# theEricMa/ScaleDreamer

Hardware: AMD Instinct MI355X
Metric: ASD train steps/sec (64x64 render, SD2.1) (higher is better)
Workload: dtype f32 renderer / f16 diffusion (f32 accumulate); 1 GPU; asd_sd_nerf: 1 view/GPU, 64x64 rays, 512 spp occgrid march, implicit-volume iNGP (16x2 hash grid 2^19, MLP 64), SD-2.1 UNet batch 5 (CFG+Perp-Neg+shifted t), VAE 512^2 fwd+bwd, AdamW; views_per_gpu=1, parallelism=dp1, diffusion_backend=hip, diffusion_weights=seeded random init (seed 1)

## Files before the change

scaledreamer_amd/csrc/nn_ops.hip:

```cpp
#include "asd_common.h"
#include <type_traits>

typedef _Float16 half_t;
typedef half_t half8 __attribute__((ext_vector_type(8)));

__device__ __forceinline__ float silu_f(float v) { return asd_silu_fast(v); }
__device__ __forceinline__ float gelu_f(float x) { return 0.5f * x * (1.f + erff(x * 0.70710678118654752440f)); }

#ifndef GN_UNR
#define GN_UNR 4
#endif
#ifndef GN_CAP_A
#define GN_CAP_A 512
#endif
#ifndef GN_FOLD_RECORDS
#define GN_FOLD_RECORDS 96
#endif

__global__ __launch_bounds__(256) void gn_stats_kernel(const half_t* __restrict__ x1, int c1, const half_t* __restrict__ x2,
                                                       int c2, int hw, int rows_per_block, float* __restrict__ stats) {
    __shared__ float gsum[32], gsq[32];
    const int C = c1 + c2, slots = C / 8, cg = C / 32;
    const int b = blockIdx.x, tid = threadIdx.x;
    if (tid < 32) { gsum[tid] = 0.f; gsq[tid] = 0.f; }
    __syncthreads();
    const int r0 = blockIdx.y * rows_per_block, r1 = min(hw, r0 + rows_per_block);
    const int rows_in_flight = slots >= 256 ? 1 : 256 / slots;
    const int rsub = slots >= 256 ? 0 : tid / slots;
    const int slot0 = slots >= 256 ? tid : tid % slots;
#pragma unroll
    for (int j = 0; j < 2; ++j) {
        const int slot = slot0 + j * 256;
        if (slot >= slots || rsub >= rows_in_flight || (j == 1 && slots <= 256)) continue;
        float s[8], q[8];
#pragma unroll
        for (int k = 0; k < 8; ++k) { s[k] = 0.f; q[k] = 0.f; }
        const int c = slot * 8;
        const half_t* base = c < c1 ? x1 + (size_t)b * hw * c1 + c : x2 + (size_t)b * hw * c2 + (c - c1);
        const size_t rstride = c < c1 ? c1 : c2;
        int r = r0 + rsub;
        for (; r + (GN_UNR - 1) * rows_in_flight < r1; r += GN_UNR * rows_in_flight) {
            half8 v[GN_UNR];
#pragma unroll
            for (int u = 0; u < GN_UNR; ++u) v[u] = *(const half8*)(base + (size_t)(r + u * rows_in_flight) * rstride);
#pragma unroll
            for (int u = 0; u < GN_UNR; ++u)
#pragma unroll
                for (int k = 0; k < 8; ++k) { const float f = (float)v[u][k]; s[k] += f; q[k] = fmaf(f, f, q[k]); }
        }
        for (; r < r1; r += rows_in_flight) {
            const half8 v = *(const half8*)(base + (size_t)r * rstride);
#pragma unroll
            for (int k = 0; k < 8; ++k) { const float f = (float)v[k]; s[k] += f; q[k] = fmaf(f, f, q[k]); }
        }
        int g = c / cg;
        float ss = 0.f, qq = 0.f;
#pragma unroll
        for (int k = 0; k < 8; ++k) {
            const int gk = (c + k) / cg;
            if (gk != g) { atomicAdd(&gsum[g], ss); atomicAdd(&gsq[g], qq); g = gk; ss = 0.f; qq = 0.f; }
            ss += s[k]; qq += q[k];
        }
        atomicAdd(&gsum[g], ss);
        atomicAdd(&gsq[g], qq);
    }
    __syncthreads();
    if (tid < 32) {
        float* part = stats + ((size_t)b * gridDim.y + blockIdx.y) * 64;
        part[tid * 2] = gsum[tid];
        part[tid * 2 + 1] = gsq[tid];
    }
}

__device__ __forceinline__ void gn_reduce_partials(const float* __restrict__ partials, int b, int n_chunks, float* st ,
                                                   float (*scratch)[64] ) {
    const int tid = threadIdx.x, v = tid & 63, q = tid >> 6;
    const float* src = partials + (size_t)b * n_chunks * 64 + v;
    float acc[8];
#pragma unroll
    for (int u = 0; u < 8; ++u) acc[u] = 0.f;
    for (int c = q; c < n_chunks; c += 32) {
        float t[8];
#pragma unroll
        for (int u = 0; u < 8; ++u) t[u] = src[(size_t)min(c + 4 * u, n_chunks - 1) * 64];
#pragma unroll
        for (int u = 0; u < 8; ++u) acc[u] += c + 4 * u < n_chunks ? t[u] : 0.f;
    }
    scratch[q][v] = ((acc[0] + acc[1]) + (acc[2] + acc[3])) + ((acc[4] + acc[5]) + (acc[6] + acc[7]));
    __syncthreads();
    if (tid < 64) st[tid] = (scratch[0][tid] + scratch[1][tid]) + (scratch[2][tid] + scratch[3][tid]);
    __syncthreads();
}

template <bool SILU>
__global__ __launch_bounds__(256) void gn_apply_kernel(const half_t* __restrict__ x1, int c1, const half_t* __restrict__ x2,
                                                       int c2, int hw, int rows_per_block, const half_t* __restrict__ gamma,
                                                       const half_t* __restrict__ beta, float eps, float inv_cnt,
                                                       const float* __restrict__ partials, int n_chunks,
                                                       float* __restrict__ stats_out, half_t* __restrict__ y) {
    __shared__ float st[64];
    __shared__ float scratch[4][64];
    const int C = c1 + c2, slots = C / 8, cg = C / 32;
    const int b = blockIdx.x, tid = threadIdx.x;
    const int r0 = blockIdx.y * rows_per_block, r1 = min(hw, r0 + rows_per_block);
    const int rows_in_flight = slots >= 256 ? 1 : 256 / slots;
    const int rsub = slots >= 256 ? 0 : tid / slots;
    const int slot0 = slots >= 256 ? tid : tid % slots;
    const bool act0 = slot0 < slots && rsub < rows_in_flight;
    const int cA = slot0 * 8;
    const half_t* baseA = cA < c1 ? x1 + (size_t)b * hw * c1 + cA : x2 + (size_t)b * hw * c2 + (cA - c1);
    const size_t rstrideA = cA < c1 ? c1 : c2;
    half8 pre[GN_UNR], gpre = {}, bpre = {};
    const int rA = r0 + rsub;
    const bool pre_ok = act0 && rA + (GN_UNR - 1) * rows_in_flight < r1;
    if (act0) { gpre = *(const half8*)(gamma + cA); bpre = *(const half8*)(beta + cA); }
    if (pre_ok) {
#pragma unroll
        for (int u = 0; u < GN_UNR; ++u) pre[u] = *(const half8*)(baseA + (size_t)(rA + u * rows_in_flight) * rstrideA);
    }
    gn_reduce_partials(partials, b, n_chunks, st, scratch);
    if (blockIdx.y == 0 && tid < 64) stats_out[b * 64 + tid] = st[tid];
#pragma unroll
    for (int j = 0; j < 2; ++j) {
        const int slot = slot0 + j * 256;
        if (slot >= slots || rsub >= rows_in_flight || (j == 1 && slots <= 256)) continue;
        const int c = slot * 8;
        half8 gv = gpre, bv = bpre;
        if (j == 1) { gv = *(const half8*)(gamma + c); bv = *(const half8*)(beta + c); }
        float sa[8], sb[8], ta[8], tb[8];
#pragma unroll
        for (int k = 0; k < 8; ++k) {
            const int g = (c + k) / cg;
            const float mean = st[g * 2] * inv_cnt;
            const float var = fmaxf(st[g * 2 + 1] * inv_cnt - mean * mean, 0.f);
            sa[k] = rsqrtf(var + eps) * (float)gv[k];
            sb[k] = (float)bv[k] - mean * sa[k];
            ta[k] = ASD_NEG_LOG2E * sa[k]; tb[k] = ASD_NEG_LOG2E * sb[k];
        }
        const half_t* base = c < c1 ? x1 + (size_t)b * hw * c1 + c : x2 + (size_t)b * hw * c2 + (c - c1);
        const size_t rstride = c < c1 ? c1 : c2;
        half_t* ybase = y + (size_t)b * hw * C + c;
        auto emit = [&](const half8& v, int r) __attribute__((always_inline)) {
            half8 o;
#pragma unroll
            for (int k = 0; k < 8; ++k) {
                const float xf = (float)v[k];
                float f = fmaf(xf, sa[k], sb[k]);
                if (SILU) f *= asd_sigmoid_exp2(fmaf(xf, ta[k], tb[k]));
                o[k] = (half_t)f;
            }
            *(half8*)(ybase + (size_t)r * C) = o;
        };
        int r = r0 + rsub;
        if (j == 0 && pre_ok) {
#pragma unroll
            for (int u = 0; u < GN_UNR; ++u) emit(pre[u], r + u * rows_in_flight);
            r += GN_UNR * rows_in_flight;
        }
        auto trips = [&](auto uc) __attribute__((always_inline)) {
            constexpr int U = decltype(uc)::value;
            for (; r + (U - 1) * rows_in_flight < r1; r += U * rows_in_flight) {
                half8 v[U];
#pragma unroll
                for (int u = 0; u < U; ++u) v[u] = *(const half8*)(base + (size_t)(r + u * rows_in_flight) * rstride);
#pragma unroll
                for (int u = 0; u < U; ++u) emit(v[u], r + u * rows_in_flight);
            }
        };
        trips(std::integral_constant<int, GN_UNR>{});
        trips(std::integral_constant<int, 1>{});
    }
}

__device__ __forceinline__ float silu_grad(float z) { return asd_silu_grad_fast(z); }

#ifndef GN_BWD_UNR
#define GN_BWD_UNR 4
#endif
#ifndef GN_BWD_WIDE_NT
#define GN_BWD_WIDE_NT 512
#endif

template <int NT, bool SILU>
__global__ __launch_bounds__(NT) void gn_bwd_stats_kernel(const half_t* __restrict__ x, const half_t* __restrict__ dy, int C,
                                                           int hw, int rows_per_block, const half_t* __restrict__ gamma,
                                                           const half_t* __restrict__ beta, float eps, float inv_cnt,
                                                           const float* __restrict__ fstats, float* __restrict__ bstats) {
    __shared__ float gsum[32], gsq[32];
    const int slots = C / 8, cg = C / 32;
    const int b = blockIdx.x, tid = threadIdx.x;
    if (tid < 32) { gsum[tid] = 0.f; gsq[tid] = 0.f; }
    __syncthreads();
    const int r0 = blockIdx.y * rows_per_block, r1 = min(hw, r0 + rows_per_block);
    const int rows_in_flight = slots >= NT ? 1 : NT / slots;
    const int rsub = slots >= NT ? 0 : tid / slots;
    const int slot0 = slots >= NT ? tid : tid % slots;
#pragma unroll
    for (int j = 0; j < 2; ++j) {
        const int slot = slot0 + j * NT;
        if (slot >= slots || rsub >= rows_in_flight || (j == 1 && slots <= NT)) continue;
        const int c = slot * 8;
        float rstd[8], nmr[8], gm[8], bt[8], s[8], q[8];
#pragma unroll
        for (int k = 0; k < 8; ++k) {
            const int g = (c + k) / cg;
            const float mean = fstats[(b * 32 + g) * 2] * inv_cnt;
            rstd[k] = rsqrtf(fmaxf(fstats[(b * 32 + g) * 2 + 1] * inv_cnt - mean * mean, 0.f) + eps);
            nmr[k] = -mean * rstd[k];
            gm[k] = (float)gamma[c + k]; bt[k] = (float)beta[c + k];
            s[k] = 0.f; q[k] = 0.f;
        }
        auto accum = [&](const half8& xv, const half8& dv) __attribute__((always_inline)) {
#pragma unroll
            for (int k = 0; k < 8; ++k) {
                const float xh = fmaf((float)xv[k], rstd[k], nmr[k]);
                float g = (float)dv[k] * gm[k];
                if (SILU) g *= silu_grad(fmaf(xh, gm[k], bt[k]));
                s[k] += g;
                q[k] = fmaf(g, xh, q[k]);
            }
        };
        int r = r0 + rsub;
        auto trips = [&](auto uc) __attribute__((always_inline)) {
            constexpr int U = decltype(uc)::value;
            for (; r + (U - 1) * rows_in_flight < r1; r += U * rows_in_flight) {
                half8 xv[U], dv[U];
#pragma unroll
                for (int u = 0; u < U; ++u) {
                    const size_t off = ((size_t)b * hw + r + u * rows_in_flight) * C + c;
                    xv[u] = *(const half8*)(x + off); dv[u] = *(const half8*)(dy + off);
                }
#pragma unroll
                for (int u = 0; u < U; ++u) accum(xv[u], dv[u]);
            }
        };
        trips(std::integral_constant<int, GN_BWD_UNR>{});
        if (GN_BWD_UNR > 2) trips(std::integral_constant<int, 2>{});
        trips(std::integral_constant<int, 1>{});
        int g = c / cg;
        float ss = 0.f, qq = 0.f;
#pragma unroll
        for (int k = 0; k < 8; ++k) {
            const int gk = (c + k) / cg;
            if (gk != g) { atomicAdd(&gsum[g], ss); atomicAdd(&gsq[g], qq); g = gk; ss = 0.f; qq = 0.f; }
            ss += s[k]; qq += q[k];
        }
        atomicAdd(&gsum[g], ss);
        atomicAdd(&gsq[g], qq);
    }
    __syncthreads();
    if (tid < 32) {
        float* part = bstats + ((size_t)b * gridDim.y + blockIdx.y) * 64;
        part[tid * 2] = gsum[tid];
        part[tid * 2 + 1] = gsq[tid];
    }
}

template <bool SILU, bool ADD>
__global__ __launch_bounds__(256) void gn_bwd_apply_kernel(const half_t* __restrict__ x, const half_t* __restrict__ dy, int C,
                                                           int hw, int rows_per_block, const half_t* __restrict__ gamma,
                                                           const half_t* __restrict__ beta, float eps, float inv_cnt,
                                                           const float* __restrict__ fstats, const float* __restrict__ bpartials,
                                                           int n_chunks, const half_t* __restrict__ dx_add,
                                                           half_t* __restrict__ dx) {
    __shared__ float st[64];
    __shared__ float scratch[4][64];
    const int slots = C / 8, cg = C / 32;
    const int b = blockIdx.x, tid = threadIdx.x;
    const int r0 = blockIdx.y * rows_per_block, r1 = min(hw, r0 + rows_per_block);
    const int rows_in_flight = slots >= 256 ? 1 : 256 / slots;
    const int rsub = slots >= 256 ? 0 : tid / slots;
    const int slot0 = slots >= 256 ? tid : tid % slots;
    const bool act0 = slot0 < slots && rsub < rows_in_flight;
    const int cA = slot0 * 8, rA = r0 + rsub;
    const bool pre_ok = act0 && rA + rows_in_flight < r1;
    half8 gpre = {}, bpre = {}, px[2], pd[2], pa[2] = {};
    if (act0) { gpre = *(const half8*)(gamma + cA); bpre = *(const half8*)(beta + cA); }
    if (pre_ok) {
#pragma unroll
        for (int u = 0; u < 2; ++u) {
            const size_t off = ((size_t)b * hw + rA + u * rows_in_flight) * C + cA;
            px[u] = *(const half8*)(x + off); pd[u] = *(const half8*)(dy + off);
            if (ADD) pa[u] = *(const half8*)(dx_add + off);
        }
    }
    gn_reduce_partials(bpartials, b, n_chunks, st, scratch);
#pragma unroll
    for (int j = 0; j < 2; ++j) {
        const int slot = slot0 + j * 256;
        if (slot >= slots || rsub >= rows_in_flight || (j == 1 && slots <= 256)) continue;
        const int c = slot * 8;
        half8 gv = gpre, bv = bpre;
        if (j == 1) { gv = *(const half8*)(gamma + c); bv = *(const half8*)(beta + c); }
        float rstd[8], nmr[8], gm[8], bt[8], G[8], c1[8], c2[8];
#pragma unroll
        for (int k = 0; k < 8; ++k) {
            const int g = (c + k) / cg;
            const float mean = fstats[(b * 32 + g) * 2] * inv_cnt;
            rstd[k] = rsqrtf(fmaxf(fstats[(b * 32 + g) * 2 + 1] * inv_cnt - mean * mean, 0.f) + eps);
            nmr[k] = -mean * rstd[k];
            gm[k] = (float)gv[k]; bt[k] = (float)bv[k];
            G[k] = gm[k] * rstd[k];
            c1[k] = -(st[g * 2] * inv_cnt) * rstd[k]; c2[k] = -(st[g * 2 + 1] * inv_cnt) * rstd[k];
        }
        auto emit = [&](const half8& xv, const half8& dv, const half8& av, int r) __attribute__((always_inline)) {
            half8 o;
#pragma unroll
            for (int k = 0; k < 8; ++k) {
                const float xh = fmaf((float)xv[k], rstd[k], nmr[k]);
                const float lin = fmaf(xh, c2[k], c1[k]);
                float f = SILU ? fmaf((float)dv[k] * G[k], silu_grad(fmaf(xh, gm[k], bt[k])), lin) : fmaf((float)dv[k], G[k], lin);
                if (ADD) f += (float)av[k];
                o[k] = (half_t)f;
            }
            *(half8*)(dx + ((size_t)b * hw + r) * C + c) = o;
        };
        int r = r0 + rsub;
        if (j == 0 && pre_ok) {
            emit(px[0], pd[0], pa[0], r);
            emit(px[1], pd[1], pa[1], r + rows_in_flight);
            r += 2 * rows_in_flight;
        }
        auto trips = [&](auto uc) __attribute__((always_inline)) {
            constexpr int U = decltype(uc)::value;
            for (; r + (U - 1) * rows_in_flight < r1; r += U * rows_in_flight) {
                half8 xv[U], dv[U], av[U] = {};
#pragma unroll
                for (int u = 0; u < U; ++u) {
                    const size_t off = ((size_t)b * hw + r + u * rows_in_flight) * C + c;
                    xv[u] = *(const half8*)(x + off); dv[u] = *(const half8*)(dy + off);
                    if (ADD) av[u] = *(const half8*)(dx_add + off);
                }
#pragma unroll
                for (int u = 0; u < U; ++u) emit(xv[u], dv[u], av[u], r + u * rows_in_flight);
            }
        };
        trips(std::integral_constant<int, GN_BWD_UNR>{});
        if (GN_BWD_UNR > 2) trips(std::integral_constant<int, 2>{});
        trips(std::integral_constant<int, 1>{});
    }
}

__global__ __launch_bounds__(256) void transpose_f16_kernel(const half_t* __restrict__ x, int rows, int cols, int ldx,
                                                            half_t* __restrict__ y, int ldy) {
    __shared__ half_t tile[64][66];
    const int r0 = blockIdx.y * 64, c0 = blockIdx.x * 64;
    for (int q = threadIdx.x; q < 64 * 64; q += 256) {
        const int r = q / 64, c = q % 64;
        tile[r][c] = (r0 + r < rows && c0 + c < cols) ? x[(size_t)(r0 + r) * ldx + c0 + c] : (half_t)0.f;
    }
    __syncthreads();
    for (int q = threadIdx.x; q < 64 * 64; q += 256) {
        const int c = q / 64, r = q % 64;
        if (c0 + c < cols && r0 + r < rows) y[(size_t)(c0 + c) * ldy + r0 + r] = tile[r][c];
    }
}

template <int NV>
__global__ __launch_bounds__(256) void layernorm_kernel(const half_t* __restrict__ x, int rows, int C,
                                                        const half_t* __restrict__ gamma, const half_t* __restrict__ beta,
                                                        float eps, half_t* __restrict__ y) {
    const int lane = threadIdx.x & 63;
    const int wave = blockIdx.x * 4 + (threadIdx.x >> 6), n_waves = gridDim.x * 4;
    half8 gm[NV], bt[NV];
#pragma unroll
    for (int j = 0; j < NV; ++j) {
        const int c = lane * 8 + j * 512;
        if (c < C) { gm[j] = *(const half8*)(gamma + c); bt[j] = *(const half8*)(beta + c); }
    }
    const float inv_c = 1.f / (float)C;
    for (int row = wave; row < rows; row += n_waves) {
        const half_t* xr = x + (size_t)row * C;
        half8 v[NV];
        float s = 0.f;
#pragma unroll
        for (int j = 0; j < NV; ++j) {
            const int c = lane * 8 + j * 512;
            if (c < C) {
                v[j] = *(const half8*)(xr + c);
#pragma unroll
                for (int k = 0; k < 8; ++k) s += (float)v[j][k];
            }
        }
        const float mean = asd_wave_sum(s) * inv_c;
        float q = 0.f;
#pragma unroll
        for (int j = 0; j < NV; ++j)
            if (lane * 8 + j * 512 < C) {
#pragma unroll
                for (int k = 0; k < 8; ++k) { const float d = (float)v[j][k] - mean; q = fmaf(d, d, q); }
            }
        const float rstd = rsqrtf(asd_wave_sum(q) * inv_c + eps);
#pragma unroll
        for (int j = 0; j < NV; ++j) {
            const int c = lane * 8 + j * 512;
            if (c < C) {
                half8 o;
#pragma unroll
                for (int k = 0; k < 8; ++k) o[k] = (half_t)(((float)v[j][k] - mean) * rstd * (float)gm[j][k] + (float)bt[j][k]);
                *(half8*)(y + (size_t)row * C + c) = o;
            }
        }
    }
}


__device__ __forceinline__ float block_reduce(float v, float* red, bool is_max) {
#pragma unroll
    for (int off = 32; off > 0; off >>= 1) {
        const float o = __shfl_xor(v, off, 64);
        v = is_max ? fmaxf(v, o) : v + o;
    }
    const int wave = threadIdx.x >> 6;
    __syncthreads();
    if ((threadIdx.x & 63) == 0) red[wave] = v;
    __syncthreads();
    const float a = red[0], b = red[1], c = red[2], d = red[3];
    return is_max ? fmaxf(fmaxf(a, b), fmaxf(c, d)) : (a + b) + (c + d);
}

template <int NV>
__global__ __launch_bounds__(256) void softmax_kernel(const half_t* __restrict__ x, int ldx, int cols, float scale,
                                                      half_t* __restrict__ y, int ldy) {
    __shared__ float red[4];
    const half_t* xr = x + (size_t)blockIdx.x * ldx;
    half8 v[NV];
    float m = -INFINITY;
#pragma unroll
    for (int j = 0; j < NV; ++j) {
        const int c = threadIdx.x * 8 + j * 2048;
        if (c < cols) {
            v[j] = *(const half8*)(xr + c);
#pragma unroll
            for (int k = 0; k < 8; ++k) m = fmaxf(m, (float)v[j][k]);
        }
    }
    m = block_reduce(m, red, true) * scale;
    float e[NV][8];
    float s = 0.f;
#pragma unroll
    for (int j = 0; j < NV; ++j)
        if (threadIdx.x * 8 + j * 2048 < cols) {
#pragma unroll
            for (int k = 0; k < 8; ++k) { e[j][k] = __expf(fmaf((float)v[j][k], scale, -m)); s += e[j][k]; }
        }
    const float inv = 1.f / block_reduce(s, red, false);
#pragma unroll
    for (int j = 0; j < NV; ++j) {
        const int c = threadIdx.x * 8 + j * 2048;
        if (c < cols) {
            half8 o;
#pragma unroll
            for (int k = 0; k < 8; ++k) o[k] = (half_t)(e[j][k] * inv);
            *(half8*)(y + (size_t)blockIdx.x * ldy + c) = o;
        }
    }
}

template <int NV>
__global__ __launch_bounds__(256) void softmax_bwd_kernel(const half_t* __restrict__ p, const half_t* __restrict__ dp, int ld,
                                                          int cols, float scale, half_t* __restrict__ ds) {
    __shared__ float red[4];
    const size_t base = (size_t)blockIdx.x * ld;
    half8 pv[NV], dv[NV];
    float s = 0.f;
#pragma unroll
    for (int j = 0; j < NV; ++j) {
        const int c = threadIdx.x * 8 + j * 2048;
        if (c < cols) {
            pv[j] = *(const half8*)(p + base + c);
            dv[j] = *(const half8*)(dp + base + c);
#pragma unroll
            for (int k = 0; k < 8; ++k) s = fmaf((float)pv[j][k], (float)dv[j][k], s);
        }
    }
    s = block_reduce(s, red, false);
#pragma unroll
    for (int j = 0; j < NV; ++j) {
        const int c = threadIdx.x * 8 + j * 2048;
        if (c < cols) {
            half8 o;
#pragma unroll
            for (int k = 0; k < 8; ++k) o[k] = (half_t)(scale * (float)pv[j][k] * ((float)dv[j][k] - s));
            *(half8*)(ds + base + c) = o;
        }
    }
}

__global__ __launch_bounds__(256) void geglu_kernel(const half_t* __restrict__ h, int rows, int C, half_t* __restrict__ y) {
    const int slots = C / 8;
    const size_t total = (size_t)rows * slots;
    for (size_t i = (size_t)blockIdx.x * 256 + threadIdx.x; i < total; i += (size_t)gridDim.x * 256) {
        const size_t row = i / slots;
        const int c = (int)(i - row * slots) * 8;
        const half8 a = *(const half8*)(h + row * 2 * C + c), g = *(const half8*)(h + row * 2 * C + C + c);
        half8 o;
#pragma unroll
        for (int k = 0; k < 8; ++k) o[k] = (half_t)((float)a[k] * gelu_f((float)g[k]));
        *(half8*)(y + row * C + c) = o;
    }
}

__global__ __launch_bounds__(256) void silu_kernel(const half_t* __restrict__ x, size_t n8, half_t* __restrict__ y) {
    for (size_t i = (size_t)blockIdx.x * 256 + threadIdx.x; i < n8; i += (size_t)gridDim.x * 256) {
        const half8 v = *(const half8*)(x + i * 8);
        half8 o;
#pragma unroll
        for (int k = 0; k < 8; ++k) o[k] = (half_t)silu_f((float)v[k]);
        *(half8*)(y + i * 8) = o;
    }
}

__global__ void timestep_embedding_kernel(const float* __restrict__ t, int n, int dim, half_t* __restrict__ y) {
    const int i = blockIdx.x * blockDim.x + threadIdx.x;
    const int half = dim / 2;
    if (i >= n * half) return;
    const int r = i / half, k = i - r * half;
    const float freq = expf(-logf(10000.f) * (float)k / (float)half);
    const float a = t[r] * freq;
    y[(size_t)r * dim + k] = (half_t)cosf(a);
    y[(size_t)r * dim + half + k] = (half_t)sinf(a);
}

__global__ __launch_bounds__(256) void concat_kernel(const half_t* __restrict__ x1, int c1, const half_t* __restrict__ x2, int c2,
                                                     size_t rows, half_t* __restrict__ y) {
    const int C = c1 + c2, slots = C / 8;
    const size_t total = rows * slots;
    for (size_t i = (size_t)blockIdx.x * 256 + threadIdx.x; i < total; i += (size_t)gridDim.x * 256) {
        const size_t row = i / slots;
        const int c = (int)(i - row * slots) * 8;
        *(half8*)(y + row * C + c) = c < c1 ? *(const half8*)(x1 + row * c1 + c) : *(const half8*)(x2 + row * c2 + (c - c1));
    }
}

__global__ __launch_bounds__(256) void pad_cast_kernel(const float* __restrict__ x, size_t rows, int c, half_t* __restrict__ y, int c_pad) {
    const size_t total = rows * (size_t)c_pad;
    for (size_t i = (size_t)blockIdx.x * 256 + threadIdx.x; i < total; i += (size_t)gridDim.x * 256) {
        const size_t r = i / c_pad;
        const int j = (int)(i - r * c_pad);
        y[i] = j < c ? (half_t)x[r * c + j] : (half_t)0.f;
    }
}

__global__ __launch_bounds__(1024) void gn_reduce_records_kernel(const float* __restrict__ records, int n, float* __restrict__ out) {
    __shared__ float scratch[16][64];
    const int b = blockIdx.x, S = gridDim.y, per = (n + S - 1) / S;
    const int c0 = blockIdx.y * per, c1 = min(n, c0 + per);
    const int v = threadIdx.x & 63, q = threadIdx.x >> 6;
    const float* src = records + (size_t)b * n * 64 + v;
    float acc[8];
#pragma unroll
    for (int u = 0; u < 8; ++u) acc[u] = 0.f;
    int c = c0 + q;
    for (; c + 7 * 16 < c1; c += 8 * 16) {
        float t[8];
#pragma unroll
        for (int u = 0; u < 8; ++u) t[u] = src[(size_t)(c + u * 16) * 64];
#pragma unroll
        for (int u = 0; u < 8; ++u) acc[u] += t[u];
    }
#pragma unroll
    for (int u = 0; u < 8; ++u)
        if (c + u * 16 < c1) acc[u] += src[(size_t)(c + u * 16) * 64];
    scratch[q][v] = ((acc[0] + acc[1]) + (acc[2] + acc[3])) + ((acc[4] + acc[5]) + (acc[6] + acc[7]));
    __syncthreads();
    if (threadIdx.x < 64) {
        float s = 0.f;
#pragma unroll
        for (int u = 0; u < 16; ++u) s += scratch[u][v];
        out[((size_t)b * S + blockIdx.y) * 64 + v] = s;
    }
}

static int gn_apply_chunks(int hw, int C, int batch) {
    const int slots = C / 8, rif = slots >= 256 ? 1 : 256 / slots;
    const int chunks = asd_div_up(hw, GN_UNR * rif), cap_a = asd_div_up(GN_CAP_A, batch);
    return chunks > cap_a ? cap_a : chunks;
}

__global__ __launch_bounds__(256) void gather_rows_kernel(const uint4* __restrict__ src, const int* __restrict__ idx, size_t row16,
                                                          uint4* __restrict__ dst) {
    const size_t i = blockIdx.y;
    const uint4* s = src + (size_t)idx[i] * row16;
    uint4* d = dst + i * row16;
    for (size_t q = (size_t)blockIdx.x * 256 + threadIdx.x; q < row16; q += (size_t)gridDim.x * 256) d[q] = s[q];
}

static void gn_launch_apply(dim3 grid, hipStream_t s, const void* x1, int c1, const void* x2, int c2, int hw, int rows_per_block,
                            const void* gamma, const void* beta, float eps, int silu, const float* partials, int n_chunks, float* stats,
                            void* y) {
    const float inv_cnt = 1.f / ((float)hw * (float)((c1 + c2) / 32));
#define GN_APPLY_ARGS (const half_t*)x1, c1, (const half_t*)x2, c2, hw, rows_per_block, (const half_t*)gamma, (const half_t*)beta, eps, inv_cnt, \
                      partials, n_chunks, stats, (half_t*)y
    if (silu) hipLaunchKernelGGL(gn_apply_kernel<true>, grid, dim3(256), 0, s, GN_APPLY_ARGS);
    else hipLaunchKernelGGL(gn_apply_kernel<false>, grid, dim3(256), 0, s, GN_APPLY_ARGS);
#undef GN_APPLY_ARGS
}

static void gn_launch_bwd_stats(bool wide, dim3 grid, hipStream_t s, const void* x, const void* dy, int c, int hw, int rows_per_block,
                                const void* gamma, const void* beta, float eps, int silu, const float* fstats, float* bstats) {
    const float inv_cnt = 1.f / ((float)hw * (float)(c / 32));
#define GN_BWD_STATS_ARGS (const half_t*)x, (const half_t*)dy, c, hw, rows_per_block, (const half_t*)gamma, (const half_t*)beta, eps, inv_cnt, fstats, bstats
    if (wide) {
        if (silu) hipLaunchKernelGGL((gn_bwd_stats_kernel<GN_BWD_WIDE_NT, true>), grid, dim3(GN_BWD_WIDE_NT), 0, s, GN_BWD_STATS_ARGS);
        else hipLaunchKernelGGL((gn_bwd_stats_kernel<GN_BWD_WIDE_NT, false>), grid, dim3(GN_BWD_WIDE_NT), 0, s, GN_BWD_STATS_ARGS);
    } else {
        if (silu) hipLaunchKernelGGL((gn_bwd_stats_kernel<256, true>), grid, dim3(256), 0, s, GN_BWD_STATS_ARGS);
        else hipLaunchKernelGGL((gn_bwd_stats_kernel<256, false>), grid, dim3(256), 0, s, GN_BWD_STATS_ARGS);
    }
#undef GN_BWD_STATS_ARGS
}

static void gn_launch_bwd_apply(dim3 grid, hipStream_t s, const void* x, const void* dy, int c, int hw, int rows_per_block, const void* gamma,
                                const void* beta, float eps, int silu, const float* fstats, const float* bpartials, int n_chunks,
                                const void* dx_add, void* dx) {
    const float inv_cnt = 1.f / ((float)hw * (float)(c / 32));
#define GN_BWD_APPLY_ARGS (const half_t*)x, (const half_t*)dy, c, hw, rows_per_block, (const half_t*)gamma, (const half_t*)beta, eps, inv_cnt, fstats, \
                          bpartials, n_chunks, (const half_t*)dx_add, (half_t*)dx
    if (silu) {
        if (dx_add) hipLaunchKernelGGL((gn_bwd_apply_kernel<true, true>), grid, dim3(256), 0, s, GN_BWD_APPLY_ARGS);
        else hipLaunchKernelGGL((gn_bwd_apply_kernel<true, false>), grid, dim3(256), 0, s, GN_BWD_APPLY_ARGS);
    } else {
        if (dx_add) hipLaunchKernelGGL((gn_bwd_apply_kernel<false, true>), grid, dim3(256), 0, s, GN_BWD_APPLY_ARGS);
        else hipLaunchKernelGGL((gn_bwd_apply_kernel<false, false>), grid, dim3(256), 0, s, GN_BWD_APPLY_ARGS);
    }
#undef GN_BWD_APPLY_ARGS
}

extern "C" {

int asd_gather_rows_f16(const void* src, const int32_t* idx_dev, int32_t n_out, int64_t row_halfs, void* dst, void* stream) {
    ASD_CHECK_ARG(src && idx_dev && dst && n_out > 0 && row_halfs > 0 && row_halfs % 8 == 0, "bad argument");
    const size_t row16 = (size_t)row_halfs / 8;
    int bx = (int)((row16 + 1023) / 1024);
    if (bx > 256) bx = 256;
    hipLaunchKernelGGL(gather_rows_kernel, dim3(bx, n_out), dim3(256), 0, (hipStream_t)stream, (const uint4*)src, (const int*)idx_dev, row16,
                       (uint4*)dst);
    ASD_LAUNCH_CHECK();
    return ASD_OK;
}

int asd_groupnorm_f16(const void* x1, int32_t c1, const void* x2, int32_t c2, int32_t batch, int32_t hw, const void* gamma,
                      const void* beta, float eps, int32_t silu, void* y, float* stats, void* stream) {
    ASD_CHECK_ARG(x1 && gamma && beta && y && stats && batch > 0 && hw > 0, "null argument");
    const int C = c1 + (x2 ? c2 : 0);
    if (!x2) c2 = 0;
    ASD_CHECK_ARG(C % 32 == 0 && C % 8 == 0 && c1 % 8 == 0, "channels must be a multiple of 32");
    ASD_CHECK_ARG(((((uintptr_t)gamma) | ((uintptr_t)beta)) & 15) == 0, "gamma / beta must be 16-byte aligned");
    hipStream_t s = (hipStream_t)stream;
    float* partials = stats + 64 * batch;
    int chunks = asd_div_up(hw, 16);
    const int cap_s = asd_div_up(256, batch);
    const int chunks_s = chunks > cap_s ? cap_s : chunks, chunks_a = gn_apply_chunks(hw, C, batch);
    hipLaunchKernelGGL(gn_stats_kernel, dim3(batch, chunks_s), dim3(256), 0, s, (const half_t*)x1, c1, (const half_t*)x2, c2, hw,
                       asd_div_up(hw, chunks_s), partials);
    gn_launch_apply(dim3(batch, chunks_a), s, x1, c1, x2, c2, hw, asd_div_up(hw, chunks_a), gamma, beta, eps, silu, partials, chunks_s, stats, y);
    ASD_LAUNCH_CHECK();
    return ASD_OK;
}

int asd_groupnorm_apply_f16(const void* x, int32_t c, int32_t batch, int32_t hw, const void* gamma, const void* beta, float eps,
                            int32_t silu, const float* partials, int32_t records, void* y, float* stats , void* stream) {
    ASD_CHECK_ARG(x && gamma && beta && y && stats && partials && batch > 0 && hw > 0 && records > 0, "null argument");
    ASD_CHECK_ARG(c % 32 == 0 && c % 8 == 0, "channels must be a multiple of 32");
    ASD_CHECK_ARG(((((uintptr_t)gamma) | ((uintptr_t)beta)) & 15) == 0, "gamma / beta must be 16-byte aligned");
    hipStream_t s = (hipStream_t)stream;
    const int chunks_a = gn_apply_chunks(hw, c, batch);
    const float* part = partials;
    int n = records;
    if (records > GN_FOLD_RECORDS) {
        int slices = asd_div_up(records, 32);
        if (slices > 16) slices = 16;
        float* tmp = stats + 64 * batch;
        hipLaunchKernelGGL(gn_reduce_records_kernel, dim3(batch, slices), dim3(1024), 0, s, partials, records, tmp);
        part = tmp;
        n = slices;
    }
    gn_launch_apply(dim3(batch, chunks_a), s, x, c, nullptr, 0, hw, asd_div_up(hw, chunks_a), gamma, beta, eps, silu, part, n, stats, y);
    ASD_LAUNCH_CHECK();
    return ASD_OK;
}

int asd_groupnorm_bwd_f16(const void* x, const void* dy, int32_t c, int32_t batch, int32_t hw, const void* gamma,
                          const void* beta, float eps, int32_t silu, const float* fwd_stats, const void* dx_add, void* dx,
                          float* bwd_stats, void* stream) {
    ASD_CHECK_ARG(x && dy && gamma && beta && fwd_stats && dx && bwd_stats && batch > 0 && hw > 0, "null argument");
    ASD_CHECK_ARG(c % 32 == 0, "channels must be a multiple of 32");
    ASD_CHECK_ARG(((((uintptr_t)gamma) | ((uintptr_t)beta)) & 15) == 0, "gamma / beta must be 16-byte aligned");
    hipStream_t s = (hipStream_t)stream;
    int chunks = asd_div_up(hw, 16);
    const int cap_s = asd_div_up(256, batch), cap_a = asd_div_up(GN_CAP_A, batch);
    const int chunks_s = chunks > cap_s ? cap_s : chunks, chunks_a = chunks > cap_a ? cap_a : chunks;
    const bool wide = (size_t)asd_div_up(hw, chunks_s) * c >= 32768 && c % 8 == 0 && GN_BWD_WIDE_NT % (c / 8) == 0;
    gn_launch_bwd_stats(wide, dim3(batch, chunks_s), s, x, dy, c, hw, asd_div_up(hw, chunks_s), gamma, beta, eps, silu, fwd_stats, bwd_stats);
    gn_launch_bwd_apply(dim3(batch, chunks_a), s, x, dy, c, hw, asd_div_up(hw, chunks_a), gamma, beta, eps, silu, fwd_stats, bwd_stats, chunks_s,
                        dx_add, dx);
    ASD_LAUNCH_CHECK();
    return ASD_OK;
}

int asd_groupnorm_bwd_apply_f16(const void* x, const void* dy, int32_t c, int32_t batch, int32_t hw, const void* gamma, const void* beta,
                                float eps, int32_t silu, const float* fwd_stats, const float* partials, int32_t records,
                                const void* dx_add, void* dx, float* scratch, void* stream) {
    ASD_CHECK_ARG(x && dy && gamma && beta && fwd_stats && partials && dx && scratch && batch > 0 && hw > 0 && records > 0, "null argument");
    ASD_CHECK_ARG(c % 32 == 0, "channels must be a multiple of 32");
    ASD_CHECK_ARG(((((uintptr_t)gamma) | ((uintptr_t)beta)) & 15) == 0, "gamma / beta must be 16-byte aligned");
    hipStream_t s = (hipStream_t)stream;
    const int chunks = asd_div_up(hw, 16);
    const int cap_a = asd_div_up(GN_CAP_A, batch), chunks_a = chunks > cap_a ? cap_a : chunks;
    const float* part = partials;
    int n = records;
    if (records > GN_FOLD_RECORDS) {
        int slices = asd_div_up(records, 32);
        if (slices > 16) slices = 16;
        hipLaunchKernelGGL(gn_reduce_records_kernel, dim3(batch, slices), dim3(1024), 0, s, partials, records, scratch);
        part = scratch;
        n = slices;
    }
    gn_launch_bwd_apply(dim3(batch, chunks_a), s, x, dy, c, hw, asd_div_up(hw, chunks_a), gamma, beta, eps, silu, fwd_stats, part, n, dx_add, dx);
    ASD_LAUNCH_CHECK();
    return ASD_OK;
}

int asd_transpose_f16(const void* x, int32_t rows, int32_t cols, int32_t ldx, void* y, int32_t ldy, void* stream) {
    ASD_CHECK_ARG(x && y && rows > 0 && cols > 0 && ldx >= cols && ldy >= rows, "bad argument");
    hipLaunchKernelGGL(transpose_f16_kernel, dim3(asd_div_up(cols, 64), asd_div_up(rows, 64)), dim3(256), 0, (hipStream_t)stream,
                       (const half_t*)x, rows, cols, ldx, (half_t*)y, ldy);
    ASD_LAUNCH_CHECK();
    return ASD_OK;
}

int asd_layernorm_f16(const void* x, int32_t rows, int32_t c, const void* gamma, const void* beta, float eps, void* y,
                      void* stream) {
    ASD_CHECK_ARG(x && gamma && beta && y && rows > 0, "null argument");
    ASD_CHECK_ARG(c % 8 == 0 && c <= 2048, "channels must be a multiple of 8 and <= 2048");
    int blocks = asd_div_up(rows, 4);
    if (blocks > 2048) blocks = 2048;
    const dim3 g(blocks), blk(256);
    hipStream_t s = (hipStream_t)stream;
#define LN_LAUNCH(NV) hipLaunchKernelGGL((layernorm_kernel<NV>), g, blk, 0, s, (const half_t*)x, rows, c, (const half_t*)gamma, \
                                         (const half_t*)beta, eps, (half_t*)y)
    if (c <= 512) LN_LAUNCH(1);
    else if (c <= 1024) LN_LAUNCH(2);
    else if (c <= 1536) LN_LAUNCH(3);
    else LN_LAUNCH(4);
#undef LN_LAUNCH
    ASD_LAUNCH_CHECK();
    return ASD_OK;
}

int asd_softmax_f16(const void* x, int32_t ldx, int32_t rows, int32_t cols, float scale, void* y, int32_t ldy, void* stream) {
    ASD_CHECK_ARG(x && y && rows > 0 && cols > 0, "null argument");
    ASD_CHECK_ARG(cols % 8 == 0 && cols <= 8192 && ldx % 8 == 0 && ldy % 8 == 0, "cols must be a multiple of 8 and <= 8192");
    const dim3 g(rows), blk(256);
    hipStream_t s = (hipStream_t)stream;
#define SM_LAUNCH(NV) hipLaunchKernelGGL((softmax_kernel<NV>), g, blk, 0, s, (const half_t*)x, ldx, cols, scale, (half_t*)y, ldy)
    if (cols <= 2048) SM_LAUNCH(1);
    else if (cols <= 4096) SM_LAUNCH(2);
    else SM_LAUNCH(4);
#undef SM_LAUNCH
    ASD_LAUNCH_CHECK();
    return ASD_OK;
}

int asd_softmax_bwd_f16(const void* p, const void* dp, int32_t ld, int32_t rows, int32_t cols, float scale, void* ds,
                        void* stream) {
    ASD_CHECK_ARG(p && dp && ds && rows > 0 && cols > 0, "null argument");
    ASD_CHECK_ARG(cols % 8 == 0 && cols <= 8192 && ld % 8 == 0, "cols must be a multiple of 8 and <= 8192");
    const dim3 g(rows), blk(256);
    hipStream_t s = (hipStream_t)stream;
#define SMB_LAUNCH(NV) hipLaunchKernelGGL((softmax_bwd_kernel<NV>), g, blk, 0, s, (const half_t*)p, (const half_t*)dp, ld, cols, scale, (half_t*)ds)
    if (cols <= 2048) SMB_LAUNCH(1);
    else if (cols <= 4096) SMB_LAUNCH(2);
    else SMB_LAUNCH(4);
#undef SMB_LAUNCH
    ASD_LAUNCH_CHECK();
    return ASD_OK;
}

int asd_geglu_f16(const void* h, int32_t rows, int32_t c, void* y, void* stream) {
    ASD_CHECK_ARG(h && y && rows > 0 && c % 8 == 0, "bad argument");
    hipLaunchKernelGGL(geglu_kernel, dim3(asd_grid_for((size_t)rows * c / 8, 256)), dim3(256), 0, (hipStream_t)stream,
                       (const half_t*)h, rows, c, (half_t*)y);
    ASD_LAUNCH_CHECK();
    return ASD_OK;
}

int asd_silu_f16(const void* x, int64_t n, void* y, void* stream) {
    ASD_CHECK_ARG(x && y && n > 0 && n % 8 == 0, "bad argument");
    hipLaunchKernelGGL(silu_kernel, dim3(asd_grid_for(n / 8, 256)), dim3(256), 0, (hipStream_t)stream, (const half_t*)x,
                       (size_t)(n / 8), (half_t*)y);
    ASD_LAUNCH_CHECK();
    return ASD_OK;
}

int asd_timestep_embedding_f16(const float* t, int32_t n, int32_t dim, void* y, void* stream) {
    ASD_CHECK_ARG(t && y && n > 0 && dim % 2 == 0, "bad argument");
    hipLaunchKernelGGL(timestep_embedding_kernel, dim3(asd_div_up(n * dim / 2, 256)), dim3(256), 0, (hipStream_t)stream, t, n,
                       dim, (half_t*)y);
    ASD_LAUNCH_CHECK();
    return ASD_OK;
}

int asd_concat_f16(const void* x1, int32_t c1, const void* x2, int32_t c2, int64_t rows, void* y, void* stream) {
    ASD_CHECK_ARG(x1 && x2 && y && rows > 0 && c1 % 8 == 0 && c2 % 8 == 0, "bad argument");
    hipLaunchKernelGGL(concat_kernel, dim3(asd_grid_for((size_t)rows * (c1 + c2) / 8, 256)), dim3(256), 0, (hipStream_t)stream,
                       (const half_t*)x1, c1, (const half_t*)x2, c2, (size_t)rows, (half_t*)y);
    ASD_LAUNCH_CHECK();
    return ASD_OK;
}

int asd_pad_cast_f16(const float* x, int32_t rows, int32_t c, void* y, int32_t c_pad, void* stream) {
    ASD_CHECK_ARG(x && y && rows > 0 && c > 0 && c_pad >= c, "bad argument");
    const size_t total = (size_t)rows * c_pad;
    hipLaunchKernelGGL(pad_cast_kernel, dim3(asd_grid_for(total, 256)), dim3(256), 0, (hipStream_t)stream, x, (size_t)rows, c, (half_t*)y, c_pad);
    ASD_LAUNCH_CHECK();
    return ASD_OK;
}

}
```

Before: 70.52 steps/s.

## Double-buffer row loads in GroupNorm kernels via shared walk helper

```diff
diff --git a/scaledreamer_amd/csrc/gn_rows.h b/scaledreamer_amd/csrc/gn_rows.h
--- /dev/null
+++ b/scaledreamer_amd/csrc/gn_rows.h
@@ -0,0 +1,89 @@
+#pragma once
+
+#if defined(__HIPCC__) || defined(__CUDACC__)
+#define GN_HD __host__ __device__ __forceinline__
+#else
+#define GN_HD inline
+#endif
+#if defined(__HIP_DEVICE_COMPILE__)
+#define GN_SCHED_FENCE() __builtin_amdgcn_sched_barrier(0)
+#else
+#define GN_SCHED_FENCE() ((void)0)
+#endif
+
+struct gn_walk {
+    int slot0;
+    int first;
+    int rif;
+    int n;
+};
+
+GN_HD gn_walk gn_walk_make(int hw, int slots, int nt, int rows_per_block, int block, int tid) {
+    gn_walk w;
+    const int r0 = block * rows_per_block, r1 = hw < r0 + rows_per_block ? hw : r0 + rows_per_block;
+    w.rif = slots >= nt ? 1 : nt / slots;
+    const int rsub = slots >= nt ? 0 : tid / slots;
+    w.slot0 = slots >= nt ? tid : tid % slots;
+    w.first = r0 + rsub;
+    w.n = (w.slot0 < slots && rsub < w.rif && w.first < r1) ? (r1 - w.first + w.rif - 1) / w.rif : 0;
+    return w;
+}
+GN_HD int gn_walk_passes(const gn_walk& w, int slots, int nt) { return w.n == 0 ? 0 : (w.slot0 + nt < slots ? 2 : 1); }
+GN_HD int gn_walk_row(const gn_walk& w, int i) { return w.first + i * w.rif; }
+GN_HD int gn_walk_tail_row(const gn_walk& w, int i, int u) { return gn_walk_row(w, i + u < w.n ? i + u : w.n - 1); }
+
+template <int U, class Buf, class Load, class Use>
+GN_HD void gn_walk_trips(const gn_walk& w, Buf& a, Load&& load, Use&& use) {
+    Buf b;
+    int i = 0;
+    for (; i + 3 * U <= w.n; i += 2 * U) {
+        load(b, i + U);
+        GN_SCHED_FENCE();
+#pragma unroll
+        for (int u = 0; u < U; ++u) use(a, i, u);
+        GN_SCHED_FENCE();
+        load(a, i + 2 * U);
+        GN_SCHED_FENCE();
+#pragma unroll
+        for (int u = 0; u < U; ++u) use(b, i + U, u);
+        GN_SCHED_FENCE();
+    }
+    auto part = [&](const Buf& t, int at) __attribute__((always_inline)) {
+#pragma unroll
+        for (int u = 0; u < U; ++u)
+            if (at + u < w.n) use(t, at, u);
+    };
+    const bool t1 = i + U < w.n, t2 = i + 2 * U < w.n;
+    if (t1) load(b, i + U);
+    part(a, i);
+    if (t2) load(a, i + 2 * U);
+    if (t1) part(b, i + U);
+    if (t2) part(a, i + 2 * U);
+}
+
+static inline int gn_div_up(int a, int b) { return (a + b - 1) / b; }
+#ifndef GN_UNR
+#define GN_UNR 4
+#endif
+#ifndef GN_BWD_UNR
+#define GN_BWD_UNR 4
+#endif
+#ifndef GN_CAP_A
+#define GN_CAP_A 512
+#endif
+#ifndef GN_CAP_S
+#define GN_CAP_S 256
+#endif
+static inline int gn_stats_chunks(int hw, int batch) {
+    const int chunks = gn_div_up(hw, 16), cap_s = gn_div_up(GN_CAP_S, batch);
+    return chunks > cap_s ? cap_s : chunks;
+}
+static inline int gn_apply_chunks(int hw, int C, int batch) {
+    const int slots = C / 8, rif = slots >= 256 ? 1 : 256 / slots;
+    const int chunks = gn_div_up(hw, GN_UNR * rif), cap_a = gn_div_up(GN_CAP_A, batch);
+    return chunks > cap_a ? cap_a : chunks;
+}
+static inline int gn_bwd_apply_chunks(int hw, int batch) {
+    const int chunks = gn_div_up(hw, 16), cap_a = gn_div_up(GN_CAP_A, batch);
+    return chunks > cap_a ? cap_a : chunks;
+}
diff --git a/scaledreamer_amd/csrc/nn_ops.hip b/scaledreamer_amd/csrc/nn_ops.hip
--- a/scaledreamer_amd/csrc/nn_ops.hip
+++ b/scaledreamer_amd/csrc/nn_ops.hip
@@ -1,5 +1,5 @@
 #include "asd_common.h"
-#include <type_traits>
+#include "gn_rows.h"
 
 typedef _Float16 half_t;
 typedef half_t half8 __attribute__((ext_vector_type(8)));
@@ -7,15 +7,27 @@
 __device__ __forceinline__ float silu_f(float v) { return asd_silu_fast(v); }
 __device__ __forceinline__ float gelu_f(float x) { return 0.5f * x * (1.f + erff(x * 0.70710678118654752440f)); }
 
-#ifndef GN_UNR
-#define GN_UNR 4
-#endif
-#ifndef GN_CAP_A
-#define GN_CAP_A 512
-#endif
 #ifndef GN_FOLD_RECORDS
 #define GN_FOLD_RECORDS 96
 #endif
+
+struct gn_buf1 { half8 v[GN_UNR]; };
+__device__ __forceinline__ void gn_load1(gn_buf1& d, const gn_walk& w, int i, const half_t* __restrict__ base, size_t rstride) {
+#pragma unroll
+    for (int u = 0; u < GN_UNR; ++u) d.v[u] = *(const half8*)(base + (size_t)gn_walk_tail_row(w, i, u) * rstride);
+}
+template <bool ADD>
+struct gn_buf3 { half8 x[GN_BWD_UNR], d[GN_BWD_UNR], a[ADD ? GN_BWD_UNR : 1]; };
+template <bool ADD>
+__device__ __forceinline__ void gn_load3(gn_buf3<ADD>& t, const gn_walk& w, int i, const half_t* __restrict__ x, const half_t* __restrict__ dy,
+                                         const half_t* __restrict__ dx_add, size_t row0, int C, int c) {
+#pragma unroll
+    for (int u = 0; u < GN_BWD_UNR; ++u) {
+        const size_t off = (row0 + gn_walk_tail_row(w, i, u)) * C + c;
+        t.x[u] = *(const half8*)(x + off); t.d[u] = *(const half8*)(dy + off);
+        if (ADD) t.a[u] = *(const half8*)(dx_add + off);
+    }
+}
 
 __global__ __launch_bounds__(256) void gn_stats_kernel(const half_t* __restrict__ x1, int c1, const half_t* __restrict__ x2,
                                                        int c2, int hw, int rows_per_block, float* __restrict__ stats) {
@@ -24,35 +36,24 @@
     const int b = blockIdx.x, tid = threadIdx.x;
     if (tid < 32) { gsum[tid] = 0.f; gsq[tid] = 0.f; }
     __syncthreads();
-    const int r0 = blockIdx.y * rows_per_block, r1 = min(hw, r0 + rows_per_block);
-    const int rows_in_flight = slots >= 256 ? 1 : 256 / slots;
-    const int rsub = slots >= 256 ? 0 : tid / slots;
-    const int slot0 = slots >= 256 ? tid : tid % slots;
+    const gn_walk w = gn_walk_make(hw, slots, 256, rows_per_block, blockIdx.y, tid);
+    const int passes = gn_walk_passes(w, slots, 256);
 #pragma unroll
     for (int j = 0; j < 2; ++j) {
-        const int slot = slot0 + j * 256;
-        if (slot >= slots || rsub >= rows_in_flight || (j == 1 && slots <= 256)) continue;
+        if (j >= passes) continue;
         float s[8], q[8];
 #pragma unroll
         for (int k = 0; k < 8; ++k) { s[k] = 0.f; q[k] = 0.f; }
-        const int c = slot * 8;
+        const int c = (w.slot0 + j * 256) * 8;
         const half_t* base = c < c1 ? x1 + (size_t)b * hw * c1 + c : x2 + (size_t)b * hw * c2 + (c - c1);
         const size_t rstride = c < c1 ? c1 : c2;
-        int r = r0 + rsub;
-        for (; r + (GN_UNR - 1) * rows_in_flight < r1; r += GN_UNR * rows_in_flight) {
-            half8 v[GN_UNR];
-#pragma unroll
-            for (int u = 0; u < GN_UNR; ++u) v[u] = *(const half8*)(base + (size_t)(r + u * rows_in_flight) * rstride);
-#pragma unroll
-            for (int u = 0; u < GN_UNR; ++u)
-#pragma unroll
-                for (int k = 0; k < 8; ++k) { const float f = (float)v[u][k]; s[k] += f; q[k] = fmaf(f, f, q[k]); }
-        }
-        for (; r < r1; r += rows_in_flight) {
-            const half8 v = *(const half8*)(base + (size_t)r * rstride);
-#pragma unroll
-            for (int k = 0; k < 8; ++k) { const float f = (float)v[k]; s[k] += f; q[k] = fmaf(f, f, q[k]); }
-        }
+        gn_buf1 first;
+        gn_load1(first, w, 0, base, rstride);
+        gn_walk_trips<GN_UNR>(w, first, [&](gn_buf1& t, int i) __attribute__((always_inline)) { gn_load1(t, w, i, base, rstride); },
+                              [&](const gn_buf1& t, int, int u) __attribute__((always_inline)) {
+#pragma unroll
+                                  for (int k = 0; k < 8; ++k) { const float f = (float)t.v[u][k]; s[k] += f; q[k] = fmaf(f, f, q[k]); }
+                              });
         int g = c / cg;
         float ss = 0.f, qq = 0.f;
 #pragma unroll
@@ -102,29 +103,21 @@
     __shared__ float scratch[4][64];
     const int C = c1 + c2, slots = C / 8, cg = C / 32;
     const int b = blockIdx.x, tid = threadIdx.x;
-    const int r0 = blockIdx.y * rows_per_block, r1 = min(hw, r0 + rows_per_block);
-    const int rows_in_flight = slots >= 256 ? 1 : 256 / slots;
-    const int rsub = slots >= 256 ? 0 : tid / slots;
-    const int slot0 = slots >= 256 ? tid : tid % slots;
-    const bool act0 = slot0 < slots && rsub < rows_in_flight;
-    const int cA = slot0 * 8;
-    const half_t* baseA = cA < c1 ? x1 + (size_t)b * hw * c1 + cA : x2 + (size_t)b * hw * c2 + (cA - c1);
-    const size_t rstrideA = cA < c1 ? c1 : c2;
-    half8 pre[GN_UNR], gpre = {}, bpre = {};
-    const int rA = r0 + rsub;
-    const bool pre_ok = act0 && rA + (GN_UNR - 1) * rows_in_flight < r1;
-    if (act0) { gpre = *(const half8*)(gamma + cA); bpre = *(const half8*)(beta + cA); }
-    if (pre_ok) {
-#pragma unroll
-        for (int u = 0; u < GN_UNR; ++u) pre[u] = *(const half8*)(baseA + (size_t)(rA + u * rows_in_flight) * rstrideA);
+    const gn_walk w = gn_walk_make(hw, slots, 256, rows_per_block, blockIdx.y, tid);
+    const int passes = gn_walk_passes(w, slots, 256);
+    const int cA = w.slot0 * 8;
+    half8 gpre = {}, bpre = {};
+    gn_buf1 first;
+    if (passes > 0) {
+        gpre = *(const half8*)(gamma + cA); bpre = *(const half8*)(beta + cA);
+        gn_load1(first, w, 0, cA < c1 ? x1 + (size_t)b * hw * c1 + cA : x2 + (size_t)b * hw * c2 + (cA - c1), cA < c1 ? c1 : c2);
     }
     gn_reduce_partials(partials, b, n_chunks, st, scratch);
     if (blockIdx.y == 0 && tid < 64) stats_out[b * 64 + tid] = st[tid];
 #pragma unroll
     for (int j = 0; j < 2; ++j) {
-        const int slot = slot0 + j * 256;
-        if (slot >= slots || rsub >= rows_in_flight || (j == 1 && slots <= 256)) continue;
-        const int c = slot * 8;
+        if (j >= passes) continue;
+        const int c = (w.slot0 + j * 256) * 8;
         half8 gv = gpre, bv = bpre;
         if (j == 1) { gv = *(const half8*)(gamma + c); bv = *(const half8*)(beta + c); }
         float sa[8], sb[8], ta[8], tb[8];
@@ -140,43 +133,24 @@
         const half_t* base = c < c1 ? x1 + (size_t)b * hw * c1 + c : x2 + (size_t)b * hw * c2 + (c - c1);
         const size_t rstride = c < c1 ? c1 : c2;
         half_t* ybase = y + (size_t)b * hw * C + c;
-        auto emit = [&](const half8& v, int r) __attribute__((always_inline)) {
-            half8 o;
-#pragma unroll
-            for (int k = 0; k < 8; ++k) {
-                const float xf = (float)v[k];
-                float f = fmaf(xf, sa[k], sb[k]);
-                if (SILU) f *= asd_sigmoid_exp2(fmaf(xf, ta[k], tb[k]));
-                o[k] = (half_t)f;
-            }
-            *(half8*)(ybase + (size_t)r * C) = o;
-        };
-        int r = r0 + rsub;
-        if (j == 0 && pre_ok) {
-#pragma unroll
-            for (int u = 0; u < GN_UNR; ++u) emit(pre[u], r + u * rows_in_flight);
-            r += GN_UNR * rows_in_flight;
-        }
-        auto trips = [&](auto uc) __attribute__((always_inline)) {
-            constexpr int U = decltype(uc)::value;
-            for (; r + (U - 1) * rows_in_flight < r1; r += U * rows_in_flight) {
-                half8 v[U];
-#pragma unroll
-                for (int u = 0; u < U; ++u) v[u] = *(const half8*)(base + (size_t)(r + u * rows_in_flight) * rstride);
-#pragma unroll
-                for (int u = 0; u < U; ++u) emit(v[u], r + u * rows_in_flight);
-            }
-        };
-        trips(std::integral_constant<int, GN_UNR>{});
-        trips(std::integral_constant<int, 1>{});
+        if (j == 1) gn_load1(first, w, 0, base, rstride);
+        gn_walk_trips<GN_UNR>(w, first, [&](gn_buf1& t, int i) __attribute__((always_inline)) { gn_load1(t, w, i, base, rstride); },
+                              [&](const gn_buf1& t, int i, int u) __attribute__((always_inline)) {
+                                  half8 o;
+#pragma unroll
+                                  for (int k = 0; k < 8; ++k) {
+                                      const float xf = (float)t.v[u][k];
+                                      float f = fmaf(xf, sa[k], sb[k]);
+                                      if (SILU) f *= asd_sigmoid_exp2(fmaf(xf, ta[k], tb[k]));
+                                      o[k] = (half_t)f;
+                                  }
+                                  *(half8*)(ybase + (size_t)gn_walk_row(w, i + u) * C) = o;
+                              });
     }
 }
 
 __device__ __forceinline__ float silu_grad(float z) { return asd_silu_grad_fast(z); }
 
-#ifndef GN_BWD_UNR
-#define GN_BWD_UNR 4
-#endif
 #ifndef GN_BWD_WIDE_NT
 #define GN_BWD_WIDE_NT 512
 #endif
@@ -191,15 +165,14 @@
     const int b = blockIdx.x, tid = threadIdx.x;
     if (tid < 32) { gsum[tid] = 0.f; gsq[tid] = 0.f; }
     __syncthreads();
-    const int r0 = blockIdx.y * rows_per_block, r1 = min(hw, r0 + rows_per_block);
-    const int rows_in_flight = slots >= NT ? 1 : NT / slots;
-    const int rsub = slots >= NT ? 0 : tid / slots;
-    const int slot0 = slots >= NT ? tid : tid % slots;
+    const gn_walk w = gn_walk_make(hw, slots, NT, rows_per_block, blockIdx.y, tid);
+    const int passes = gn_walk_passes(w, slots, NT);
 #pragma unroll
     for (int j = 0; j < 2; ++j) {
-        const int slot = slot0 + j * NT;
-        if (slot >= slots || rsub >= rows_in_flight || (j == 1 && slots <= NT)) continue;
-        const int c = slot * 8;
+        if (j >= passes) continue;
+        const int c = (w.slot0 + j * NT) * 8;
+        gn_buf3<false> first;
+        gn_load3<false>(first, w, 0, x, dy, nullptr, (size_t)b * hw, C, c);
         float rstd[8], nmr[8], gm[8], bt[8], s[8], q[8];
 #pragma unroll
         for (int k = 0; k < 8; ++k) {
@@ -210,33 +183,18 @@
             gm[k] = (float)gamma[c + k]; bt[k] = (float)beta[c + k];
             s[k] = 0.f; q[k] = 0.f;
         }
-        auto accum = [&](const half8& xv, const half8& dv) __attribute__((always_inline)) {
-#pragma unroll
-            for (int k = 0; k < 8; ++k) {
-                const float xh = fmaf((float)xv[k], rstd[k], nmr[k]);
-                float g = (float)dv[k] * gm[k];
-                if (SILU) g *= silu_grad(fmaf(xh, gm[k], bt[k]));
-                s[k] += g;
-                q[k] = fmaf(g, xh, q[k]);
-            }
-        };
-        int r = r0 + rsub;
-        auto trips = [&](auto uc) __attribute__((always_inline)) {
-            constexpr int U = decltype(uc)::value;
-            for (; r + (U - 1) * rows_in_flight < r1; r += U * rows_in_flight) {
-                half8 xv[U], dv[U];
-#pragma unroll
-                for (int u = 0; u < U; ++u) {
-                    const size_t off = ((size_t)b * hw + r + u * rows_in_flight) * C + c;
-                    xv[u] = *(const half8*)(x + off); dv[u] = *(const half8*)(dy + off);
-                }
-#pragma unroll
-                for (int u = 0; u < U; ++u) accum(xv[u], dv[u]);
-            }
-        };
-        trips(std::integral_constant<int, GN_BWD_UNR>{});
-        if (GN_BWD_UNR > 2) trips(std::integral_constant<int, 2>{});
-        trips(std::integral_constant<int, 1>{});
+        gn_walk_trips<GN_BWD_UNR>(w, first,
+                                  [&](gn_buf3<false>& t, int i) __attribute__((always_inline)) { gn_load3<false>(t, w, i, x, dy, nullptr, (size_t)b * hw, C, c); },
+                                  [&](const gn_buf3<false>& t, int, int u) __attribute__((always_inline)) {
+#pragma unroll
+                                      for (int k = 0; k < 8; ++k) {
+                                          const float xh = fmaf((float)t.x[u][k], rstd[k], nmr[k]);
+                                          float g = (float)t.d[u][k] * gm[k];
+                                          if (SILU) g *= silu_grad(fmaf(xh, gm[k], bt[k]));
+                                          s[k] += g;
+                                          q[k] = fmaf(g, xh, q[k]);
+                                      }
+                                  });
         int g = c / cg;
         float ss = 0.f, qq = 0.f;
 #pragma unroll
@@ -267,31 +225,25 @@
     __shared__ float scratch[4][64];
     const int slots = C / 8, cg = C / 32;
     const int b = blockIdx.x, tid = threadIdx.x;
-    const int r0 = blockIdx.y * rows_per_block, r1 = min(hw, r0 + rows_per_block);
-    const int rows_in_flight = slots >= 256 ? 1 : 256 / slots;
-    const int rsub = slots >= 256 ? 0 : tid / slots;
-    const int slot0 = slots >= 256 ? tid : tid % slots;
-    const bool act0 = slot0 < slots && rsub < rows_in_flight;
-    const int cA = slot0 * 8, rA = r0 + rsub;
-    const bool pre_ok = act0 && rA + rows_in_flight < r1;
-    half8 gpre = {}, bpre = {}, px[2], pd[2], pa[2] = {};
-    if (act0) { gpre = *(const half8*)(gamma + cA); bpre = *(const half8*)(beta + cA); }
-    if (pre_ok) {
-#pragma unroll
-        for (int u = 0; u < 2; ++u) {
-            const size_t off = ((size_t)b * hw + rA + u * rows_in_flight) * C + cA;
-            px[u] = *(const half8*)(x + off); pd[u] = *(const half8*)(dy + off);
-            if (ADD) pa[u] = *(const half8*)(dx_add + off);
-        }
+    const gn_walk w = gn_walk_make(hw, slots, 256, rows_per_block, blockIdx.y, tid);
+    const int passes = gn_walk_passes(w, slots, 256);
+    const int cA = w.slot0 * 8;
+    half8 gpre = {}, bpre = {};
+    gn_buf3<ADD> first;
+    if (passes > 0) {
+        gpre = *(const half8*)(gamma + cA); bpre = *(const half8*)(beta + cA);
+        gn_load3<ADD>(first, w, 0, x, dy, dx_add, (size_t)b * hw, C, cA);
     }
     gn_reduce_partials(bpartials, b, n_chunks, st, scratch);
 #pragma unroll
     for (int j = 0; j < 2; ++j) {
-        const int slot = slot0 + j * 256;
-        if (slot >= slots || rsub >= rows_in_flight || (j == 1 && slots <= 256)) continue;
-        const int c = slot * 8;
+        if (j >= passes) continue;
+        const int c = (w.slot0 + j * 256) * 8;
         half8 gv = gpre, bv = bpre;
-        if (j == 1) { gv = *(const half8*)(gamma + c); bv = *(const half8*)(beta + c); }
+        if (j == 1) {
+            gv = *(const half8*)(gamma + c); bv = *(const half8*)(beta + c);
+            gn_load3<ADD>(first, w, 0, x, dy, dx_add, (size_t)b * hw, C, c);
+        }
         float rstd[8], nmr[8], gm[8], bt[8], G[8], c1[8], c2[8];
 #pragma unroll
         for (int k = 0; k < 8; ++k) {
@@ -303,41 +255,21 @@
             G[k] = gm[k] * rstd[k];
             c1[k] = -(st[g * 2] * inv_cnt) * rstd[k]; c2[k] = -(st[g * 2 + 1] * inv_cnt) * rstd[k];
         }
-        auto emit = [&](const half8& xv, const half8& dv, const half8& av, int r) __attribute__((always_inline)) {
-            half8 o;
-#pragma unroll
-            for (int k = 0; k < 8; ++k) {
-                const float xh = fmaf((float)xv[k], rstd[k], nmr[k]);
-                const float lin = fmaf(xh, c2[k], c1[k]);
-                float f = SILU ? fmaf((float)dv[k] * G[k], silu_grad(fmaf(xh, gm[k], bt[k])), lin) : fmaf((float)dv[k], G[k], lin);
-                if (ADD) f += (float)av[k];
-                o[k] = (half_t)f;
-            }
-            *(half8*)(dx + ((size_t)b * hw + r) * C + c) = o;
-        };
-        int r = r0 + rsub;
-        if (j == 0 && pre_ok) {
-            emit(px[0], pd[0], pa[0], r);
-            emit(px[1], pd[1], pa[1], r + rows_in_flight);
-            r += 2 * rows_in_flight;
-        }
-        auto trips = [&](auto uc) __attribute__((always_inline)) {
-            constexpr int U = decltype(uc)::value;
-            for (; r + (U - 1) * rows_in_flight < r1; r += U * rows_in_flight) {
-                half8 xv[U], dv[U], av[U] = {};
-#pragma unroll
-                for (int u = 0; u < U; ++u) {
-                    const size_t off = ((size_t)b * hw + r + u * rows_in_flight) * C + c;
-                    xv[u] = *(const half8*)(x + off); dv[u] = *(const half8*)(dy + off);
-                    if (ADD) av[u] = *(const half8*)(dx_add + off);
-                }
-#pragma unroll
-                for (int u = 0; u < U; ++u) emit(xv[u], dv[u], av[u], r + u * rows_in_flight);
-            }
-        };
-        trips(std::integral_constant<int, GN_BWD_UNR>{});
-        if (GN_BWD_UNR > 2) trips(std::integral_constant<int, 2>{});
-        trips(std::integral_constant<int, 1>{});
+        gn_walk_trips<GN_BWD_UNR>(w, first,
+                                  [&](gn_buf3<ADD>& t, int i) __attribute__((always_inline)) { gn_load3<ADD>(t, w, i, x, dy, dx_add, (size_t)b * hw, C, c); },
+                                  [&](const gn_buf3<ADD>& t, int i, int u) __attribute__((always_inline)) {
+                                      half8 o;
+#pragma unroll
+                                      for (int k = 0; k < 8; ++k) {
+                                          const float xh = fmaf((float)t.x[u][k], rstd[k], nmr[k]);
+                                          const float lin = fmaf(xh, c2[k], c1[k]);
+                                          float f = SILU ? fmaf((float)t.d[u][k] * G[k], silu_grad(fmaf(xh, gm[k], bt[k])), lin)
+                                                         : fmaf((float)t.d[u][k], G[k], lin);
+                                          if (ADD) f += (float)t.a[u][k];
+                                          o[k] = (half_t)f;
+                                      }
+                                      *(half8*)(dx + ((size_t)b * hw + gn_walk_row(w, i + u)) * C + c) = o;
+                                  });
     }
 }
 
@@ -570,12 +502,6 @@
         for (int u = 0; u < 16; ++u) s += scratch[u][v];
         out[((size_t)b * S + blockIdx.y) * 64 + v] = s;
     }
-}
-
-static int gn_apply_chunks(int hw, int C, int batch) {
-    const int slots = C / 8, rif = slots >= 256 ? 1 : 256 / slots;
-    const int chunks = asd_div_up(hw, GN_UNR * rif), cap_a = asd_div_up(GN_CAP_A, batch);
-    return chunks > cap_a ? cap_a : chunks;
 }
 
 __global__ __launch_bounds__(256) void gather_rows_kernel(const uint4* __restrict__ src, const int* __restrict__ idx, size_t row16,
@@ -649,9 +575,7 @@
     ASD_CHECK_ARG(((((uintptr_t)gamma) | ((uintptr_t)beta)) & 15) == 0, "gamma / beta must be 16-byte aligned");
     hipStream_t s = (hipStream_t)stream;
     float* partials = stats + 64 * batch;
-    int chunks = asd_div_up(hw, 16);
-    const int cap_s = asd_div_up(256, batch);
-    const int chunks_s = chunks > cap_s ? cap_s : chunks, chunks_a = gn_apply_chunks(hw, C, batch);
+    const int chunks_s = gn_stats_chunks(hw, batch), chunks_a = gn_apply_chunks(hw, C, batch);
     hipLaunchKernelGGL(gn_stats_kernel, dim3(batch, chunks_s), dim3(256), 0, s, (const half_t*)x1, c1, (const half_t*)x2, c2, hw,
                        asd_div_up(hw, chunks_s), partials);
     gn_launch_apply(dim3(batch, chunks_a), s, x1, c1, x2, c2, hw, asd_div_up(hw, chunks_a), gamma, beta, eps, silu, partials, chunks_s, stats, y);
@@ -688,9 +612,7 @@
     ASD_CHECK_ARG(c % 32 == 0, "channels must be a multiple of 32");
     ASD_CHECK_ARG(((((uintptr_t)gamma) | ((uintptr_t)beta)) & 15) == 0, "gamma / beta must be 16-byte aligned");
     hipStream_t s = (hipStream_t)stream;
-    int chunks = asd_div_up(hw, 16);
-    const int cap_s = asd_div_up(256, batch), cap_a = asd_div_up(GN_CAP_A, batch);
-    const int chunks_s = chunks > cap_s ? cap_s : chunks, chunks_a = chunks > cap_a ? cap_a : chunks;
+    const int chunks_s = gn_stats_chunks(hw, batch), chunks_a = gn_bwd_apply_chunks(hw, batch);
     const bool wide = (size_t)asd_div_up(hw, chunks_s) * c >= 32768 && c % 8 == 0 && GN_BWD_WIDE_NT % (c / 8) == 0;
     gn_launch_bwd_stats(wide, dim3(batch, chunks_s), s, x, dy, c, hw, asd_div_up(hw, chunks_s), gamma, beta, eps, silu, fwd_stats, bwd_stats);
     gn_launch_bwd_apply(dim3(batch, chunks_a), s, x, dy, c, hw, asd_div_up(hw, chunks_a), gamma, beta, eps, silu, fwd_stats, bwd_stats, chunks_s,
@@ -706,8 +628,7 @@
     ASD_CHECK_ARG(c % 32 == 0, "channels must be a multiple of 32");
     ASD_CHECK_ARG(((((uintptr_t)gamma) | ((uintptr_t)beta)) & 15) == 0, "gamma / beta must be 16-byte aligned");
     hipStream_t s = (hipStream_t)stream;
-    const int chunks = asd_div_up(hw, 16);
-    const int cap_a = asd_div_up(GN_CAP_A, batch), chunks_a = chunks > cap_a ? cap_a : chunks;
+    const int chunks_a = gn_bwd_apply_chunks(hw, batch);
     const float* part = partials;
     int n = records;
     if (records > GN_FOLD_RECORDS) {
```

Result: no change. 70.25 steps/s (-0.4%).
